# kdsuneraavinash/CH-Bin

Measured on AMD Instinct MI355X. Metric: convex-hull QP distances/sec (+ end-to-end bin-assign wall-clock), N=100000 D=136 B=64, higher is better.
Workload: dtype f64

## Files before the change

### ch-bin_amd/csrc/qp_kernels.hip

```cpp
#include "chb_internal.h"
#include "hull_solve16.h"
#include <cstdlib>
#include <type_traits>
#include <vector>

#include <math.h>

#include <algorithm>

#ifndef CHB_QP_UNROLL
#define CHB_QP_UNROLL 1
#endif

namespace chb {
namespace {


template <int M>
struct Sym {
    static constexpr int NP = M * (M + 1) / 2;
    __device__ static constexpr int at(int i, int j) { return i >= j ? i * (i + 1) / 2 + j : j * (j + 1) / 2 + i; }
};

template <int M>
__device__ __forceinline__ bool solve_affine(const double (&Q)[Sym<M>::NP], double s, unsigned S,
                                             double (&beta)[M])
{
    double L[M * (M - 1) / 2 + 1];
    double dg[M];
    bool ok = true;
#pragma unroll
    for (int k = 0; k < M; ++k) {
        const bool ink = (S >> k) & 1u;
        const double akk = ink ? Q[Sym<M>::at(k, k)] + s : 1.0;
        double dk = akk;
#pragma unroll
        for (int j = 0; j < k; ++j) dk -= L[k * (k - 1) / 2 + j] * L[k * (k - 1) / 2 + j] * dg[j];
        if (ink && !(dk > 1e-13 * akk)) ok = false;
        dg[k] = dk;
        const double inv = 1.0 / dk;
#pragma unroll
        for (int i = k + 1; i < M; ++i) {
            const bool ini = (S >> i) & 1u;
            double v = (ink && ini) ? Q[Sym<M>::at(i, k)] + s : 0.0;
#pragma unroll
            for (int j = 0; j < k; ++j) v -= L[i * (i - 1) / 2 + j] * L[k * (k - 1) / 2 + j] * dg[j];
            L[i * (i - 1) / 2 + k] = v * inv;
        }
    }
    if (!ok) return false;
    double z[M];
#pragma unroll
    for (int i = 0; i < M; ++i) {
        double v = ((S >> i) & 1u) ? 1.0 : 0.0;
#pragma unroll
        for (int j = 0; j < i; ++j) v -= L[i * (i - 1) / 2 + j] * z[j];
        z[i] = v;
    }
#pragma unroll
    for (int i = 0; i < M; ++i) z[i] = z[i] / dg[i];
    double sum = 0.0;
#pragma unroll
    for (int i = M - 1; i >= 0; --i) {
        double v = z[i];
#pragma unroll
        for (int j = i + 1; j < M; ++j) v -= L[j * (j - 1) / 2 + i] * beta[j];
        beta[i] = v;
        sum += v;
    }
    const double inv = 1.0 / sum;
#pragma unroll
    for (int i = 0; i < M; ++i) beta[i] *= inv;
    return sum > 0.0;
}

template <int M>
__device__ __forceinline__ double min_norm_point(const double (&Q)[Sym<M>::NP], int m,
                                                 double (&alpha)[M])
{
    double scale = 0.0;
    int i0 = 0;
    double best = kInf;
#pragma unroll
    for (int i = 0; i < M; ++i) {
        alpha[i] = 0.0;
        if (i < m) {
            const double qii = Q[Sym<M>::at(i, i)];
            scale = fmax(scale, qii);
            if (qii < best) { best = qii; i0 = i; }
        }
    }
    if (!(scale > 0.0)) {
#pragma unroll
        for (int i = 0; i < M; ++i) alpha[i] = (i == 0) ? 1.0 : 0.0;
        return scale == 0.0 ? 0.0 : scale;
    }
    unsigned S = 1u << i0, banned = 0u;
#pragma unroll
    for (int i = 0; i < M; ++i) alpha[i] = (i == i0) ? 1.0 : 0.0;
    const double tol = 1.4210854715202004e-14 * scale;

    for (int it = 0; it < 3 * M + 8; ++it) {
        double g[M];
        double val = 0.0;
#pragma unroll
        for (int i = 0; i < M; ++i) {
            double gi = 0.0;
#pragma unroll
            for (int j = 0; j < M; ++j) gi += Q[Sym<M>::at(i, j)] * alpha[j];
            g[i] = gi;
            val += alpha[i] * gi;
        }
        int jb = -1;
        double gmin = kInf;
#pragma unroll
        for (int i = 0; i < M; ++i)
            if (i < m && !(((S | banned) >> i) & 1u) && g[i] < gmin) { gmin = g[i]; jb = i; }
        if (jb < 0 || !(gmin < val - tol)) break;
        S |= 1u << jb;
        for (int mi = 0; mi <= M; ++mi) {
            double beta[M];
            if (!solve_affine<M>(Q, scale, S, beta)) {
                S &= ~(1u << jb);
                banned |= 1u << jb;
                break;
            }
            bool allpos = true;
#pragma unroll
            for (int i = 0; i < M; ++i)
                if (((S >> i) & 1u) && !(beta[i] > 0.0)) allpos = false;
            if (allpos) {
#pragma unroll
                for (int i = 0; i < M; ++i) alpha[i] = ((S >> i) & 1u) ? beta[i] : 0.0;
                break;
            }
            double theta = 1.0;
            int kr = -1;
#pragma unroll
            for (int i = 0; i < M; ++i)
                if (((S >> i) & 1u) && !(beta[i] > 0.0)) {
                    const double den = alpha[i] - beta[i];
                    const double r = den > 0.0 ? alpha[i] / den : 0.0;
                    if (kr < 0 || r < theta) { theta = r; kr = i; }
                }
#pragma unroll
            for (int i = 0; i < M; ++i) {
                const double v = alpha[i] + theta * (beta[i] - alpha[i]);
                alpha[i] = (((S >> i) & 1u) && i != kr) ? v : 0.0;
            }
            S &= ~(1u << kr);
            if (kr == jb) banned |= 1u << jb;
        }
    }
    double val = 0.0;
#pragma unroll
    for (int i = 0; i < M; ++i) {
        double gi = 0.0;
#pragma unroll
        for (int j = 0; j < M; ++j) gi += Q[Sym<M>::at(i, j)] * alpha[j];
        val += alpha[i] * gi;
    }
    return val;
}

template <int M>
__device__ __forceinline__ double affine_min_norm(const double (&Q)[Sym<M>::NP], int m, double (&alpha)[M])
{
    double scale = 0.0;
#pragma unroll
    for (int i = 0; i < M; ++i) {
        alpha[i] = 0.0;
        if (i < m) scale = fmax(scale, Q[Sym<M>::at(i, i)]);
    }
    if (!(scale > 0.0)) {
#pragma unroll
        for (int i = 0; i < M; ++i) alpha[i] = (i == 0) ? 1.0 : 0.0;
        return scale == 0.0 ? 0.0 : scale;
    }
    unsigned S = 0u;
    double beta[M];
#pragma unroll
    for (int k = 0; k < M; ++k) {
        if (k < m) {
            double trial[M];
            if (solve_affine<M>(Q, scale, S | (1u << k), trial)) {
                S |= 1u << k;
#pragma unroll
                for (int i = 0; i < M; ++i) beta[i] = trial[i];
            }
        }
    }
    if (S == 0u) {
#pragma unroll
        for (int i = 0; i < M; ++i) alpha[i] = (i == 0) ? 1.0 : 0.0;
        return Q[0];
    }
    double val = 0.0;
#pragma unroll
    for (int i = 0; i < M; ++i) alpha[i] = ((S >> i) & 1u) ? beta[i] : 0.0;
#pragma unroll
    for (int i = 0; i < M; ++i) {
        double gi = 0.0;
#pragma unroll
        for (int j = 0; j < M; ++j) gi += Q[Sym<M>::at(i, j)] * alpha[j];
        val += alpha[i] * gi;
    }
    return val;
}


__device__ __forceinline__ double reduce_scatter16(const double (&v)[16], int l16)
{
    double t8[8], t4[4], t2[2];
    const bool b8 = l16 & 8, b4 = l16 & 4, b2 = l16 & 2, b1 = l16 & 1;
#pragma unroll
    for (int e = 0; e < 8; ++e) t8[e] = (b8 ? v[e + 8] : v[e]) + __shfl_xor(b8 ? v[e] : v[e + 8], 8, 64);
#pragma unroll
    for (int e = 0; e < 4; ++e) t4[e] = (b4 ? t8[e + 4] : t8[e]) + __shfl_xor(b4 ? t8[e] : t8[e + 4], 4, 64);
#pragma unroll
    for (int e = 0; e < 2; ++e) t2[e] = (b2 ? t4[e + 2] : t4[e]) + __shfl_xor(b2 ? t4[e] : t4[e + 2], 2, 64);
    return (b1 ? t2[1] : t2[0]) + __shfl_xor(b1 ? t2[0] : t2[1], 1, 64);
}

template <int M, int WAVES, bool INDEXED>
__global__ __launch_bounds__(64 * WAVES, (M <= 5 ? 4 : 1)) void hull_qp_kernel(QpArgs a, int nprob, const int *xq,
                                                              const int *xhull, const int *xn,
                                                              int xm, double *xdist, double *xalpha, Gate gate)
{
    CHB_GATE(gate);
    constexpr int NP = Sym<M>::NP;
    static_assert(M <= 8, "m > 8 runs on hull_qp16_kernel");
    __shared__ double sQ[WAVES][NP][65];
    __shared__ int sN[WAVES][64];

    const int lane = threadIdx.x & 63, w = threadIdx.x >> 6;
    const int m = INDEXED ? xm : a.m;
    const int *act = INDEXED ? nullptr : a.active;
    if (act != nullptr) nprob = *a.n_active;
    const int npass = act != nullptr ? 1 : 16;
    const int ppw = 4 * npass;

    for (int g0 = (blockIdx.x * WAVES + w) * ppw; g0 < nprob; g0 += (int)gridDim.x * WAVES * ppw) {
    {
        const int grp = lane >> 4, l16 = lane & 15;
        for (int pass = 0; pass < npass; ++pass) {
            const int pl = pass * 4 + grp;
            const int g = g0 + pl;
            const bool valid = g < nprob;
            int n = 0, idm = -1, qid = 0;
            size_t slot = 0;
            if (valid) {
                if (INDEXED) {
                    qid = xq[g];
                    n = xn[g];
                    if (l16 < n) idm = xhull[(size_t)g * m + l16];
                } else {
                    const int pr = act ? act[g] : g;
                    const int pos = a.pos_begin + pr / a.B, c = pr - (pr / a.B) * a.B;
                    qid = a.bq[pos];
                    slot = (size_t)c * a.Kcap + pos;
                    n = a.lists.cnt[slot];
                    if (l16 < n) idm = a.lists.idx[slot * m + l16];
                }
            }
            bool changed = valid;
            if (!INDEXED && a.prev.idx != nullptr && act == nullptr && valid)
                changed = a.prev.cnt[slot] != n || (l16 < n && a.prev.idx[slot * m + l16] != idm);
            const bool doit = ((__ballot(changed) >> (16 * grp)) & 0xFFFFull) != 0ull;
            const double *vrow[M];
#pragma unroll
            for (int v = 0; v < M; ++v) {
                const int idv = __shfl(idm, 16 * grp + v, 64);
                vrow[v] = a.X + (size_t)(idv >= 0 ? idv : qid) * a.Dp;
            }
            if (!valid) continue;
            if (!doit) {
                if (l16 == 0) sN[w][pl] = -1;
                continue;
            }
            const double *xrow = a.X + (size_t)qid * a.Dp;
            double acc[NP];
#pragma unroll
            for (int e = 0; e < NP; ++e) acc[e] = 0.0;
            if (n > 0) {
                const int Dmain = a.Dp & ~31;
#pragma unroll CHB_QP_UNROLL
                for (int k = 2 * l16; k < Dmain; k += 32) {
                    const double2 xk = *reinterpret_cast<const double2 *>(xrow + k);
                    double2 y[M];
#pragma unroll
                    for (int v = 0; v < M; ++v) {
                        const double2 pv = *reinterpret_cast<const double2 *>(vrow[v] + k);
                        y[v] = double2{pv.x - xk.x, pv.y - xk.y};
                    }
#pragma unroll
                    for (int i = 0; i < M; ++i)
#pragma unroll
                        for (int j = 0; j <= i; ++j) {
                            double acc_ij = acc[Sym<M>::at(i, j)];
                            acc_ij = fma(y[i].x, y[j].x, acc_ij);
                            acc[Sym<M>::at(i, j)] = fma(y[i].y, y[j].y, acc_ij);
                        }
                }
                for (int k = Dmain + l16; k < a.Dp; k += 16) {
                    const double xk = xrow[k];
                    double y[M];
#pragma unroll
                    for (int v = 0; v < M; ++v) y[v] = vrow[v][k] - xk;
#pragma unroll
                    for (int i = 0; i < M; ++i)
#pragma unroll
                        for (int j = 0; j <= i; ++j) acc[Sym<M>::at(i, j)] = fma(y[i], y[j], acc[Sym<M>::at(i, j)]);
                }
            }
#pragma unroll
            for (int e0 = 0; e0 < NP; e0 += 16) {
                double v16[16];
#pragma unroll
                for (int e = 0; e < 16; ++e) v16[e] = e0 + e < NP ? acc[e0 + e] : 0.0;
                const double r = reduce_scatter16(v16, l16);
                if (e0 + l16 < NP) sQ[w][e0 + l16][pl] = r;
            }
            if (l16 == 0) sN[w][pl] = n;
        }
    }
    __builtin_amdgcn_wave_barrier();
    __builtin_amdgcn_s_waitcnt(0xC07F);

    const int g = g0 + lane;
    if (lane >= ppw || g >= nprob) continue;
    double Q[NP];
#pragma unroll
    for (int e = 0; e < NP; ++e) Q[e] = sQ[w][e][lane];
    const int n = sN[w][lane];
    if (n == -1) continue;
    double alpha[M];
    double dist;
    if (n <= 0) {
        dist = kInf;
#pragma unroll
        for (int v = 0; v < M; ++v) alpha[v] = 0.0;
    } else {
        const double val = a.metric == 0 ? min_norm_point<M>(Q, n, alpha) : affine_min_norm<M>(Q, n, alpha);
        dist = sqrt(fmax(val, 0.0));
    }
    if (INDEXED) {
        xdist[g] = dist;
        if (xalpha) {
#pragma unroll
            for (int v = 0; v < M; ++v)
                if (v < m) xalpha[(size_t)g * m + v] = alpha[v];
        }
    } else {
        const int pr = act ? act[g] : g;
        const int pos = a.pos_begin + pr / a.B, c = pr - (pr / a.B) * a.B;
        a.dist[(size_t)pos * a.B + c] = dist;
    }
    }
}

constexpr double kTieRel = 1e-11;

template <int CC, int NR, bool OFF32>
__device__ __forceinline__ void gram_rows(const double *X, int Dp, int Dk, int qid, int idm, int gbase, int l16,
                                          double (&r)[NR])
{
    constexpr int NP = CC * (CC + 1) / 2;
    static_assert(NP <= 16 * NR, "result registers");
    const char *Xb = reinterpret_cast<const char *>(X);
    const double *xrow = X + (size_t)qid * Dp;
    const unsigned xoff = (unsigned)qid * (unsigned)Dp * 8u;
    const double *vrow[OFF32 ? 1 : CC];
    unsigned voff[OFF32 ? CC : 1];
#pragma unroll
    for (int v = 0; v < CC; ++v) {
        const int idv = __shfl(idm, gbase + v, 64);
        if (OFF32) voff[v] = (unsigned)(idv >= 0 ? idv : qid) * (unsigned)Dp * 8u;
        else vrow[v] = X + (size_t)(idv >= 0 ? idv : qid) * Dp;
    }
    auto xat = [&](int k) { return OFF32 ? reinterpret_cast<const double *>(Xb + (size_t)(xoff + 8u * (unsigned)k)) : xrow + k; };
    auto vat = [&](int v, int k) {
        return OFF32 ? reinterpret_cast<const double *>(Xb + (size_t)(voff[OFF32 ? v : 0] + 8u * (unsigned)k)) : vrow[OFF32 ? 0 : v] + k;
    };
    double acc[NP];
#pragma unroll
    for (int e = 0; e < NP; ++e) acc[e] = 0.0;
    const int Dmain = Dk & ~31;
#pragma unroll 1
    for (int k = 2 * l16; k < Dmain; k += 32) {
        const double2 xk = *reinterpret_cast<const double2 *>(xat(k));
        double2 y[CC];
#pragma unroll
        for (int v = 0; v < CC; ++v) {
            const double2 pv = *reinterpret_cast<const double2 *>(vat(v, k));
            y[v] = double2{pv.x - xk.x, pv.y - xk.y};
        }
#pragma unroll
        for (int i = 0; i < CC; ++i)
#pragma unroll
            for (int j = 0; j <= i; ++j) {
                double t = acc[i * (i + 1) / 2 + j];
                t = fma(y[i].x, y[j].x, t);
                acc[i * (i + 1) / 2 + j] = fma(y[i].y, y[j].y, t);
            }
    }
    for (int k = Dmain + l16; k < Dk; k += 16) {
        const double xk = *xat(k);
        double y[CC];
#pragma unroll
        for (int v = 0; v < CC; ++v) y[v] = *vat(v, k) - xk;
#pragma unroll
        for (int i = 0; i < CC; ++i)
#pragma unroll
            for (int j = 0; j <= i; ++j) acc[i * (i + 1) / 2 + j] = fma(y[i], y[j], acc[i * (i + 1) / 2 + j]);
    }
#pragma unroll
    for (int t = 0; t < NR; ++t) {
        double v16[16];
#pragma unroll
        for (int e = 0; e < 16; ++e) v16[e] = 16 * t + e < NP ? acc[16 * t + e] : 0.0;
        r[t] = 16 * t < NP ? reduce_scatter16(v16, l16) : 0.0;
    }
}

#ifndef CHB_FUSED_C
#define CHB_FUSED_C 7
#endif
#ifndef CHB_FUSED_OCC
#define CHB_FUSED_OCC 3
#endif
#ifndef CHB_FUSED_WIDE
#define CHB_FUSED_WIDE 16
#endif
constexpr int kFusedWide = CHB_FUSED_WIDE;

template <bool OFF32>
__device__ __forceinline__ double diag_rows8(const double *X, int Dp, int Dk, int qid, int idm, int gbase, int l16, int v0)
{
    const char *Xb = reinterpret_cast<const char *>(X);
    const double *xrow = X + (size_t)qid * Dp;
    const unsigned xoff = (unsigned)qid * (unsigned)Dp * 8u;
    const double *vrow[OFF32 ? 1 : 8];
    unsigned voff[OFF32 ? 8 : 1];
#pragma unroll
    for (int v = 0; v < 8; ++v) {
        const int idv = __shfl(idm, gbase + v0 + v, 64);
        if (OFF32) voff[v] = (unsigned)(idv >= 0 ? idv : qid) * (unsigned)Dp * 8u;
        else vrow[v] = X + (size_t)(idv >= 0 ? idv : qid) * Dp;
    }
    auto xat = [&](int k) { return OFF32 ? reinterpret_cast<const double *>(Xb + (size_t)(xoff + 8u * (unsigned)k)) : xrow + k; };
    auto vat = [&](int v, int k) {
        return OFF32 ? reinterpret_cast<const double *>(Xb + (size_t)(voff[OFF32 ? v : 0] + 8u * (unsigned)k)) : vrow[OFF32 ? 0 : v] + k;
    };
    double acc[16];
#pragma unroll
    for (int e = 0; e < 16; ++e) acc[e] = 0.0;
    const int Dmain = Dk & ~31;
#pragma unroll 1
    for (int k = 2 * l16; k < Dmain; k += 32) {
        const double2 xk = *reinterpret_cast<const double2 *>(xat(k));
#pragma unroll
        for (int v = 0; v < 8; ++v) {
            const double2 pv = *reinterpret_cast<const double2 *>(vat(v, k));
            const double dx = pv.x - xk.x, dy = pv.y - xk.y;
            acc[v] = fma(dy, dy, fma(dx, dx, acc[v]));
        }
    }
    for (int k = Dmain + l16; k < Dk; k += 16) {
        const double xk = *xat(k);
#pragma unroll
        for (int v = 0; v < 8; ++v) {
            const double d = *vat(v, k) - xk;
            acc[v] = fma(d, d, acc[v]);
        }
    }
    return reduce_scatter16(acc, l16);
}

constexpr int kTrimMax = 32;
constexpr int kTrimKeep = 8;
constexpr int kNbTrimmed = -1;
constexpr double kTrimSlack = 1e-6;
constexpr double kTrimGamma = 2.5e-5;

__device__ __forceinline__ int trim_tail_col(int l16) { return 128 + 2 * l16; }

__device__ __forceinline__ double shadow_dot16(const unsigned short *Gs, int Dz, int qid, int ids, int nmax, int gbase, int l16,
                                               const uint4 &qm, unsigned qt)
{
    using f16x2 = __attribute__((ext_vector_type(2))) _Float16;
    auto dot2 = [](unsigned x, unsigned y, float c) {
        return __builtin_amdgcn_fdot2(__builtin_bit_cast(f16x2, x), __builtin_bit_cast(f16x2, y), c, false);
    };
    const int tcol = min(trim_tail_col(l16), Dz - 2);
    double acc[16];
#pragma unroll
    for (int v = 0; v < 16; ++v) acc[v] = 0.0;
#pragma unroll
    for (int v0 = 0; v0 < 16; v0 += 4) {
        if (v0 < nmax) {
#pragma unroll
            for (int v = v0; v < v0 + 4; ++v) {
                const int idv = __shfl(ids, gbase + v, 64);
                const unsigned short *row = Gs + (size_t)(idv >= 0 ? idv : qid) * Dz;
                const uint4 u = *reinterpret_cast<const uint4 *>(row + 8 * l16);
                const unsigned ut = *reinterpret_cast<const unsigned *>(row + tcol);
                acc[v] = (double)dot2(ut, qt, dot2(u.w, qm.w, dot2(u.z, qm.z, dot2(u.y, qm.y, dot2(u.x, qm.x, 0.f)))));
            }
        }
    }
    return reduce_scatter16(acc, l16);
}

__device__ __forceinline__ bool fused_pair_of(const FusedArgs &a, int g0, int lane, int nprob, int &pos, int &c)
{
    if (!a.stripe) {
        const int g = g0 + lane;
        pos = a.pos_begin + g / a.B;
        c = g - (g / a.B) * a.B;
        return g < nprob;
    }
    const int x = (int)(blockIdx.x & 7);
    const int nbx = (a.B - x + 7) >> 3;
    const int t = g0 + lane;
    const int pq = t / nbx;
    pos = a.pos_begin + pq;
    c = x + 8 * (t - pq * nbx);
    return pq < a.pos_end - a.pos_begin;
}

template <int M, int C, int WAVES, bool OFF32>
__global__ __launch_bounds__(64 * WAVES, CHB_FUSED_OCC) void hull_select_qp_kernel(FusedArgs a, int nprob, Gate gate)
{
    CHB_GATE(gate);
    constexpr int NPM = Sym<M>::NP;
    constexpr int NPC = C * (C + 1) / 2;
    constexpr int NR = (NPC + 15) / 16;
    constexpr int NCLS = C - M + 1;
    static_assert(C <= 8 && M <= C && C - M <= 3, "candidate Gram in registers");
    __shared__ double sQ[WAVES][NPM][65];
    __shared__ double sT[WAVES][4][NR * 16];
    __shared__ double sTh[WAVES][4][2];
    __shared__ int sSel[WAVES][4][16];
    __shared__ int sN[WAVES][64];
    __shared__ int sOrd[WAVES][64];
    __shared__ int sSlowN, sSlowBase;
    __shared__ int sTrim[WAVES][64][kTrimKeep];
    __shared__ int sTrimN[WAVES][64];
    __shared__ int sTrimCtr[3];

    const int lane = threadIdx.x & 63, w = threadIdx.x >> 6;
    const int grp = lane >> 4, l16 = lane & 15, gbase = lane & 48;
    const int m = a.m;
    const int Dk = (a.D + 7) & ~7;
    if (threadIdx.x == 0) sSlowN = 0;
    if (threadIdx.x < 3) sTrimCtr[threadIdx.x] = 0;
    __syncthreads();
    const int g0 = ((a.stripe ? (int)(blockIdx.x >> 3) : (int)blockIdx.x) * WAVES + w) * 64;
    unsigned long long slowmask = 0ull;
    int pos = 0, c = 0;
    bool valid = false;

    if (g0 < nprob) {
        valid = fused_pair_of(a, g0, lane, nprob, pos, c);
        int nb = 0, nu = 0, qid = 0;
        size_t slot = 0;
        bool changed = valid;
        if (valid) {
            qid = a.bq[pos];
            slot = (size_t)c * a.Kcap + pos;
            nb = a.cand_cnt[slot];
            if (a.candu != nullptr) nu = a.candu_cnt[slot];
            if (a.candp != nullptr && a.candp_cnt[slot] == nu) {
                if (nu == 0) changed = false;
                else if (nu <= 8) {
                    bool same = true;
                    for (int i = 0; i < nu; ++i) {
                        const int u = a.candu[slot * kCandCapU + i];
                        bool f = false;
                        for (int j = 0; j < nu; ++j) f = f || a.candp[slot * kCandCapU + j] == u;
                        same = same && f;
                    }
                    changed = !same;
                }
            }
        }
        if (a.short_cnt != nullptr) {
            bool sh = false;
            if (valid) sh = nb < min(m, a.bin_size != nullptr ? a.bin_size[c] : a.bin_ptr[c + 1] - a.bin_ptr[c]);
            const unsigned long long shm = __ballot(sh);
            if (shm != 0ull && lane == 0) atomicAdd(a.short_cnt, __popcll(shm));
        }
        int n = nb + nu;
        if (a.trim != nullptr) {
            const bool tr = changed && n > C && n <= kTrimMax;
            const unsigned long long tmask = __ballot(tr);
            const int ntrim = __popcll(tmask);
            if (ntrim > 0) {
                sTrimN[w][lane] = 0;
                if (tr) sOrd[w][__popcll(tmask & ((1ull << lane) - 1ull))] = lane;
                __builtin_amdgcn_wave_barrier();
                __builtin_amdgcn_s_waitcnt(0xC07F);
                const TrimArgs ta = *a.trim;
                auto mask32 = [](int nv) { return (unsigned)((1ull << min(max(16 * nv, 0), 32)) - 1ull); };
                const int nv = a.D - 8 * l16;
                const uint4 msk{mask32(nv), mask32(nv - 2), mask32(nv - 4), mask32(nv - 6)};
                const unsigned mskt = mask32(a.D - trim_tail_col(l16));
                int c_pairs = 0, c_in = 0, c_kept = 0;
                for (int p0 = 0; p0 < ntrim; p0 += 4) {
                    const int op = p0 + grp;
                    const bool has = op < ntrim;
                    const int pl = has ? sOrd[w][op] : 0;
                    const int n_s = __shfl(n, pl, 64);
                    const int n_g = has ? n_s : 0;
                    const int nb_g = __shfl(nb, pl, 64);
                    const int qid_g = __shfl(qid, pl, 64);
                    const size_t slot_g = (size_t)__shfl(c, pl, 64) * a.Kcap + (size_t)__shfl(pos, pl, 64);
                    int id0 = -1, id1 = -1;
                    if (l16 < n_g)
                        id0 = l16 < nb_g ? a.cand[slot_g * kCandCap + l16] : a.candu[slot_g * kCandCapU + (l16 - nb_g)];
                    if (16 + l16 < n_g)
                        id1 = 16 + l16 < nb_g ? a.cand[slot_g * kCandCap + 16 + l16] : a.candu[slot_g * kCandCapU + (16 + l16 - nb_g)];
                    bool bad = false;
                    if ((unsigned)id0 >= (unsigned)a.n_samples && id0 != -1) { bad = true; id0 = -1; }
                    if ((unsigned)id1 >= (unsigned)a.n_samples && id1 != -1) { bad = true; id1 = -1; }
                    int nmax = n_g;
                    nmax = max(nmax, __shfl_xor(nmax, 16, 64));
                    nmax = max(nmax, __shfl_xor(nmax, 32, 64));
                    nmax = __builtin_amdgcn_readfirstlane(nmax);
                    const unsigned short *qrow = ta.Gs + (size_t)qid_g * ta.Dz;
                    uint4 qm = *reinterpret_cast<const uint4 *>(qrow + 8 * l16);
                    qm.x &= msk.x; qm.y &= msk.y; qm.z &= msk.z; qm.w &= msk.w;
                    const unsigned qt = *reinterpret_cast<const unsigned *>(qrow + min(trim_tail_col(l16), ta.Dz - 2)) & mskt;
                    const float2 gj = ta.gq[qid_g];
                    const bool in0 = id0 >= 0, in1 = id1 >= 0;
                    const float2 g0 = ta.gq[in0 ? id0 : qid_g], g1 = ta.gq[in1 ? id1 : qid_g];
                    const double dot0 = shadow_dot16(ta.Gs, ta.Dz, qid_g, id0, nmax, gbase, l16, qm, qt);
                    double dot1 = 0.0;
                    if (nmax > 16) dot1 = shadow_dot16(ta.Gs, ta.Dz, qid_g, id1, nmax - 16, gbase, l16, qm, qt);
                    const double Nj = (double)gj.x, sNj = sqrt(Nj), flush = 0x1p-13 * sqrt((double)a.D);
                    auto bounds = [&](double dot, float2 gp, double &lo, double &hi) {
                        const double Np = (double)gp.x, sNp = sqrt(Np), rho = (double)gj.y + (double)gp.y;
                        const double T = Nj + Np - 2.0 * dot;
                        const double E = 2.0 * kTrimGamma * sNj * sNp + 0x1p-23 * (Nj + Np) + flush * (sNj + sNp) + 0x1p-27 * (double)a.D;
                        lo = sqrt(fmax(T - E, 0.0)) - rho;
                        hi = sqrt(T + E) + rho;
                    };
                    double lo0, lo1, hi0, hi1;
                    bounds(dot0, g0, lo0, hi0);
                    bounds(dot1, g1, lo1, hi1);
                    if (!in0) hi0 = kInf;
                    if (!in1) hi1 = kInf;
                    bad = bad || (in0 && !(hi0 < kInf)) || (in1 && !(hi1 < kInf));
                    int rank0 = 0, rank1 = 0;
#pragma unroll
                    for (int u = 0; u < 16; ++u) {
                        const double hu = __shfl(hi0, gbase + u, 64);
                        rank0 += (hu < hi0 || (hu == hi0 && u < l16)) ? 1 : 0;
                        rank1 += hu <= hi1 ? 1 : 0;
                    }
                    if (nmax > 16) {
#pragma unroll
                        for (int u = 0; u < 16; ++u) {
                            const double hu = __shfl(hi1, gbase + u, 64);
                            rank0 += hu < hi0 ? 1 : 0;
                            rank1 += (hu < hi1 || (hu == hi1 && u < l16)) ? 1 : 0;
                        }
                    }
                    double tau = (in0 && rank0 == m - 1) ? hi0 : (in1 && rank1 == m - 1) ? hi1 : kInf;
#pragma unroll
                    for (int off = 1; off < 16; off <<= 1) tau = fmin(tau, __shfl_xor(tau, off, 64));
                    const double lim = tau * (1.0 + kTrimSlack);
                    const bool k0 = in0 && !(lo0 > lim), k1 = in1 && !(lo1 > lim);
                    const unsigned badm = (unsigned)(__ballot(bad) >> gbase) & 0xffffu;
                    const unsigned b0 = (unsigned)(__ballot(k0) >> gbase) & 0xffffu, b1 = (unsigned)(__ballot(k1) >> gbase) & 0xffffu;
                    const int nk = badm != 0u ? n_g : __popc(b0) + __popc(b1);
                    if (has && badm == 0u && nk <= kTrimKeep) {
                        if (k0) sTrim[w][pl][__popc(b0 & ((1u << l16) - 1u))] = id0;
                        if (k1) sTrim[w][pl][__popc(b0) + __popc(b1 & ((1u << l16) - 1u))] = id1;
                        if (l16 == 0) sTrimN[w][pl] = nk;
                    }
                    if (has && l16 == 0) { c_pairs += 1; c_in += n_g; c_kept += nk; }
                }
                c_pairs += __shfl_xor(c_pairs, 16, 64); c_pairs += __shfl_xor(c_pairs, 32, 64);
                c_in += __shfl_xor(c_in, 16, 64); c_in += __shfl_xor(c_in, 32, 64);
                c_kept += __shfl_xor(c_kept, 16, 64); c_kept += __shfl_xor(c_kept, 32, 64);
                if (lane == 0) { atomicAdd(&sTrimCtr[0], c_pairs); atomicAdd(&sTrimCtr[1], c_in); atomicAdd(&sTrimCtr[2], c_kept); }
                __builtin_amdgcn_wave_barrier();
                __builtin_amdgcn_s_waitcnt(0xC07F);
                const int nt = sTrimN[w][lane];
                if (nt > 0) { n = nt; nb = kNbTrimmed; }
            }
        }
        int cls = 0;
        if (changed && n > 0) {
            if (n <= C) cls = n <= M ? 1 : n - M + 1;
            else if (n <= kFusedWide) cls = NCLS + 1;
        }
        slowmask = __ballot(changed && n > kFusedWide);
        sN[w][lane] = (changed && n == 0) ? 0 : -1;
        int before = 0, nwork = 0, nnarrow = 0;
#pragma unroll
        for (int k = 1; k <= NCLS + 1; ++k) {
            const unsigned long long mk = __ballot(cls == k);
            if (cls == k) before = nwork + __popcll(mk & ((1ull << lane) - 1ull));
            nwork += __popcll(mk);
            if (k == NCLS) nnarrow = nwork;
        }
        if (cls > 0) sOrd[w][before] = lane;
        __builtin_amdgcn_wave_barrier();
        __builtin_amdgcn_s_waitcnt(0xC07F);

        for (int p0 = 0; p0 < nnarrow; p0 += 4) {
            const int op = p0 + grp;
            const bool has = op < nnarrow;
            const int pl = has ? sOrd[w][op] : 0;
            const int n_s = __shfl(n, pl, 64);
            const int n_g = has ? n_s : 0;
            const int nb_g = __shfl(nb, pl, 64);
            const int qid_g = __shfl(qid, pl, 64);
            const size_t slot_g = (size_t)__shfl(c, pl, 64) * a.Kcap + (size_t)__shfl(pos, pl, 64);
            int idm = -1;
            if (l16 < n_g)
                idm = nb_g == kNbTrimmed ? sTrim[w][pl][l16]
                      : l16 < nb_g ? a.cand[slot_g * kCandCap + l16] : a.candu[slot_g * kCandCapU + (l16 - nb_g)];
            if ((unsigned)idm >= (unsigned)a.n_samples && idm != -1) {
                if (a.short_cnt != nullptr) atomicAdd(a.short_cnt, 1);
                idm = -1;
            }
            const int cw = __builtin_amdgcn_readfirstlane(__shfl(n, sOrd[w][min(p0 + 3, nnarrow - 1)], 64));
            double r[NR];
            if (cw <= M) gram_rows<M, NR, OFF32>(a.X, a.Dp, Dk, qid_g, idm, gbase, l16, r);
            else if (C >= M + 1 && cw == M + 1) gram_rows<(C >= M + 1 ? M + 1 : M), NR, OFF32>(a.X, a.Dp, Dk, qid_g, idm, gbase, l16, r);
            else if (C >= M + 2 && cw == M + 2) gram_rows<(C >= M + 2 ? M + 2 : M), NR, OFF32>(a.X, a.Dp, Dk, qid_g, idm, gbase, l16, r);
            else gram_rows<C, NR, OFF32>(a.X, a.Dp, Dk, qid_g, idm, gbase, l16, r);
            bool tie = false;
            if (has && n_g <= m) {
#pragma unroll
                for (int t = 0; t < NR; ++t)
                    if (16 * t + l16 < NPM) sQ[w][16 * t + l16][pl] = r[t];
                if (l16 == 0) sN[w][pl] = n_g;
            } else if (has) {
#pragma unroll
                for (int t = 0; t < NR; ++t) sT[w][grp][16 * t + l16] = r[t];
                __builtin_amdgcn_wave_barrier();
                __builtin_amdgcn_s_waitcnt(0xC07F);
                if (l16 < C) sSel[w][grp][8 + l16] = idm;
                __builtin_amdgcn_wave_barrier();
                __builtin_amdgcn_s_waitcnt(0xC07F);
                const double sv = l16 < n_g ? sT[w][grp][l16 * (l16 + 3) / 2] : kInf;
                int rank = 0;
#pragma unroll
                for (int u = 0; u < C; ++u) {
                    const double su = sT[w][grp][u * (u + 3) / 2];
                    const int iu = sSel[w][grp][8 + u];
                    rank += (u < n_g && u != l16 && (su < sv || (su == sv && iu < idm))) ? 1 : 0;
                }
                if (l16 < n_g) {
                    if (rank < m) sSel[w][grp][rank] = l16;
                    if (rank == m - 1) sTh[w][grp][0] = sv;
                    if (rank == m) sTh[w][grp][1] = sv;
                }
                __builtin_amdgcn_wave_barrier();
                __builtin_amdgcn_s_waitcnt(0xC07F);
                const double t0 = sTh[w][grp][0], t1 = sTh[w][grp][1];
                tie = !(t1 - t0 > kTieRel * t1);
                if (!tie) {
#pragma unroll
                    for (int t = 0; 16 * t < NPM; ++t) {
                        const int e = 16 * t + l16;
                        int i = 0;
#pragma unroll
                        for (int q = 1; q < M; ++q) i += (q * (q + 1) / 2 <= e) ? 1 : 0;
                        const int j = e - i * (i + 1) / 2;
                        if (e < NPM) {
                            double val = 0.0;
                            if (i < m) {
                                const int vi = sSel[w][grp][i], vj = sSel[w][grp][j];
                                const int hi = vi > vj ? vi : vj, lo = vi > vj ? vj : vi;
                                val = sT[w][grp][hi * (hi + 1) / 2 + lo];
                            }
                            sQ[w][e][pl] = val;
                        }
                    }
                    if (l16 == 0) sN[w][pl] = m;
                }
            }
            if (l16 == 0 && tie) slowmask |= 1ull << pl;
        }

        for (int p0 = nnarrow; p0 < nwork; p0 += 4) {
            const int op = p0 + grp;
            const bool has = op < nwork;
            const int pl = has ? sOrd[w][op] : 0;
            const int n_s = __shfl(n, pl, 64);
            const int n_g = has ? n_s : 0;
            const int nb_g = __shfl(nb, pl, 64);
            const int qid_g = __shfl(qid, pl, 64);
            const size_t slot_g = (size_t)__shfl(c, pl, 64) * a.Kcap + (size_t)__shfl(pos, pl, 64);
            int idm = -1;
            if (l16 < n_g)
                idm = nb_g == kNbTrimmed ? sTrim[w][pl][l16]
                      : l16 < nb_g ? a.cand[slot_g * kCandCap + l16] : a.candu[slot_g * kCandCapU + (l16 - nb_g)];
            if ((unsigned)idm >= (unsigned)a.n_samples && idm != -1) {
                if (a.short_cnt != nullptr) atomicAdd(a.short_cnt, 1);
                idm = -1;
            }
            int nmax = n_g;
            nmax = max(nmax, __shfl_xor(nmax, 16, 64));
            nmax = max(nmax, __shfl_xor(nmax, 32, 64));
            nmax = __builtin_amdgcn_readfirstlane(nmax);
            double sv = diag_rows8<OFF32>(a.X, a.Dp, Dk, qid_g, idm, gbase, l16, 0);
            if (nmax > 8) {
                const double s_hi = diag_rows8<OFF32>(a.X, a.Dp, Dk, qid_g, idm, gbase, l16, 8);
                const double moved = __shfl(s_hi, gbase + (l16 & 7), 64);
                sv = l16 < 8 ? sv : moved;
            }
            if (l16 >= n_g) sv = kInf;
            int rank = 0;
#pragma unroll
            for (int u = 0; u < 16; ++u) {
                const double su = __shfl(sv, gbase + u, 64);
                const int iu = __shfl(idm, gbase + u, 64);
                rank += (u < n_g && u != l16 && (su < sv || (su == sv && iu < idm))) ? 1 : 0;
            }
            if (has && l16 < n_g) {
                if (rank < m) sSel[w][grp][rank] = idm;
                if (rank == m - 1) sTh[w][grp][0] = sv;
                if (rank == m) sTh[w][grp][1] = sv;
            }
            __builtin_amdgcn_wave_barrier();
            __builtin_amdgcn_s_waitcnt(0xC07F);
            bool tie = false;
            int idm2 = -1;
            if (has) {
                const double t0 = sTh[w][grp][0], t1 = sTh[w][grp][1];
                tie = !(t1 - t0 > kTieRel * t1);
                if (l16 < m) idm2 = sSel[w][grp][l16];
            }
            double r[NR];
            gram_rows<M, NR, OFF32>(a.X, a.Dp, Dk, qid_g, idm2, gbase, l16, r);
            if (has && !tie) {
#pragma unroll
                for (int t = 0; t < NR; ++t)
                    if (16 * t + l16 < NPM) sQ[w][16 * t + l16][pl] = r[t];
                if (l16 == 0) sN[w][pl] = m;
            }
            if (l16 == 0 && tie) slowmask |= 1ull << pl;
        }
    }
    unsigned long long sm = slowmask;
    sm |= __shfl_xor(sm, 16, 64);
    sm |= __shfl_xor(sm, 32, 64);
    sm = __shfl(sm, 0, 64);
    __builtin_amdgcn_wave_barrier();
    __builtin_amdgcn_s_waitcnt(0xC07F);

    {
        const int n = valid ? sN[w][lane] : -1;
        if (valid && n != -1 && !((sm >> lane) & 1ull)) {
            double Q[NPM];
#pragma unroll
            for (int e = 0; e < NPM; ++e) Q[e] = sQ[w][e][lane];
            double alpha[M];
            double dist;
            if (n <= 0) {
                dist = kInf;
            } else {
                const double val = a.metric == 0 ? min_norm_point<M>(Q, n, alpha) : affine_min_norm<M>(Q, n, alpha);
                dist = sqrt(fmax(val, 0.0));
            }
            a.dist[(size_t)pos * a.B + c] = dist;
        }
    }

    const int nsl = __popcll(sm);
    int wbase = 0;
    if (lane == 0 && nsl > 0) wbase = atomicAdd(&sSlowN, nsl);
    __syncthreads();
    if (threadIdx.x == 0) sSlowBase = sSlowN > 0 ? atomicAdd(a.n_slow, sSlowN) : 0;
    if (threadIdx.x < 3 && a.trim != nullptr && sTrimCtr[0] > 0)
        atomicAdd(a.trim->ctr + threadIdx.x, (unsigned long long)sTrimCtr[threadIdx.x]);
    __syncthreads();
    wbase = __shfl(wbase, 0, 64) + sSlowBase;
    if (nsl > 0 && ((sm >> lane) & 1ull)) {
        const int before = __popcll(sm & ((1ull << lane) - 1ull));
        a.slow[wbase + before] = (pos - a.pos_begin) * a.B + c;
    }
}


#ifdef CHB_DEV_CLK
__device__ unsigned long long g_qp16_clk[131072][8];
#endif
#ifdef CHB_DEV_CLK
#define QP16_CLK(t) const unsigned long long t = __builtin_readcyclecounter()
#define QP16_CLK_ADD(i, v) do { if (lane == 0) atomicAdd(&g_qp16_stats[i], (unsigned long long)(v)); } while (0)
#define QP16_CLK_ACC(var, v) do { var += (unsigned long long)(v); } while (0)
#else
#define QP16_CLK(t) do { } while (0)
#define QP16_CLK_ADD(i, v) do { } while (0)
#define QP16_CLK_ACC(var, v) do { } while (0)
#endif

constexpr int kExtraMax = 2;
constexpr int kExtraNP = kExtraMax * (kExtraMax + 1) / 2;
#ifndef CHB_SW0
#define CHB_SW0 160
#define CHB_SW1 48
#define CHB_SW2 32
#endif
template <int NE, int CH, bool FULL>
__device__ __forceinline__ void gram_sweep16_chunk(const double *vptr, const double *const (&eptr)[kExtraMax],
                                                   const double *xs, int k0, int kq, int Dp, f64x4 &acc,
                                                   double (&ae)[kExtraMax], double (&ee)[kExtraNP])
{
    constexpr int NG = CH / 16;
    double2 v[NG][2], e[NE > 0 ? NE : 1][NG][2];
#pragma unroll
    for (int g = 0; g < NG; ++g) {
        const bool in = FULL || k0 + 16 * g + 4 * kq < Dp;
        v[g][0] = in ? *reinterpret_cast<const double2 *>(vptr + k0 + 16 * g) : double2{0.0, 0.0};
        v[g][1] = in ? *reinterpret_cast<const double2 *>(vptr + k0 + 16 * g + 2) : double2{0.0, 0.0};
#pragma unroll
        for (int b = 0; b < NE; ++b) {
            e[b][g][0] = in ? *reinterpret_cast<const double2 *>(eptr[b] + k0 + 16 * g) : double2{0.0, 0.0};
            e[b][g][1] = in ? *reinterpret_cast<const double2 *>(eptr[b] + k0 + 16 * g + 2) : double2{0.0, 0.0};
        }
    }
#pragma unroll
    for (int g = 0; g < NG; ++g) {
        if (FULL || k0 + 16 * g < Dp) {
            const double2 x0 = *reinterpret_cast<const double2 *>(xs + k0 + 16 * g + 4 * kq);
            const double2 x1 = *reinterpret_cast<const double2 *>(xs + k0 + 16 * g + 4 * kq + 2);
            const double y[4] = {v[g][0].x - x0.x, v[g][0].y - x0.y, v[g][1].x - x1.x, v[g][1].y - x1.y};
#pragma unroll
            for (int t = 0; t < 4; ++t) acc = __builtin_amdgcn_mfma_f64_16x16x4f64(y[t], y[t], acc, 0, 0, 0);
            double z[NE > 0 ? NE : 1][4];
#pragma unroll
            for (int b = 0; b < NE; ++b) {
                z[b][0] = e[b][g][0].x - x0.x; z[b][1] = e[b][g][0].y - x0.y;
                z[b][2] = e[b][g][1].x - x1.x; z[b][3] = e[b][g][1].y - x1.y;
#pragma unroll
                for (int t = 0; t < 4; ++t) ae[b] = fma(y[t], z[b][t], ae[b]);
#pragma unroll
                for (int b2 = 0; b2 <= b; ++b2)
#pragma unroll
                    for (int t = 0; t < 4; ++t) ee[b * (b + 1) / 2 + b2] = fma(z[b][t], z[b2][t], ee[b * (b + 1) / 2 + b2]);
            }
        }
    }
}
template <int NE, int CH>
__device__ __forceinline__ void gram_sweep16(const double *X, int Dp, int Dk, int q, int idv, const int (&ide)[kExtraMax], int kq,
                                             const double *xs, f64x4 &acc, double (&ae)[kExtraMax],
                                             double (&ee)[kExtraNP], int c0 = 0, bool first = true, bool last = true)
{
    const double *vptr = X + (size_t)(idv >= 0 ? idv : q) * Dp + 4 * kq + c0;
    const double *eptr[kExtraMax];
#pragma unroll
    for (int b = 0; b < kExtraMax; ++b) eptr[b] = X + (size_t)(b < NE ? ide[b] : q) * Dp + 4 * kq + c0;
    if (first) {
#pragma unroll
        for (int b = 0; b < kExtraMax; ++b) ae[b] = 0.0;
#pragma unroll
        for (int e = 0; e < kExtraNP; ++e) ee[e] = 0.0;
    }
    int k0 = 0;
    for (; k0 + CH <= Dk; k0 += CH) gram_sweep16_chunk<NE, CH, true>(vptr, eptr, xs, k0, kq, Dk, acc, ae, ee);
    if (k0 < Dk) gram_sweep16_chunk<NE, CH, false>(vptr, eptr, xs, k0, kq, Dk, acc, ae, ee);
    if (NE > 0 && last) {
#pragma unroll
        for (int b = 0; b < NE; ++b) {
            ae[b] += __shfl_xor(ae[b], 16, 64);
            ae[b] += __shfl_xor(ae[b], 32, 64);
        }
#pragma unroll
        for (int e = 0; e < NE * (NE + 1) / 2; ++e) {
            ee[e] += __shfl_xor(ee[e], 16, 64);
            ee[e] += __shfl_xor(ee[e], 32, 64);
        }
    }
}

template <bool INDEXED>
__global__ __launch_bounds__(256, CHB_QP16_OCC) void hull_qp16_kernel(QpArgs a, int nprob, const int *xq, const int *xhull,
                                                        const int *xn, int xm, double *xdist, double *xalpha, Gate gate)
{
    CHB_GATE(gate);
    __shared__ __attribute__((aligned(16))) double sQ[4][4][16][kQ16Ld];
    __shared__ __attribute__((aligned(16))) double sV[4][4][16];
    const int lane = threadIdx.x & 63, w = threadIdx.x >> 6;
    const int grp = lane >> 4, l16 = lane & 15;
    const int m = INDEXED ? xm : a.m;
    const int *act = INDEXED ? nullptr : a.active;
    if (act != nullptr) nprob = *a.n_active;
    for (int gw = (blockIdx.x * 4 + w) * 4; gw < nprob; gw += (int)gridDim.x * 16) {
        const int g = gw + grp;
        const bool valid = g < nprob;
        int n = 0, idm = -1, qid = 0, pr = 0;
        size_t slot = 0;
        if (valid) {
            if (INDEXED) {
                qid = xq[g];
                n = xn[g];
                if (l16 < n) idm = xhull[(size_t)g * m + l16];
            } else {
                pr = act ? act[g] : g;
                const int pos = a.pos_begin + pr / a.B, c = pr - (pr / a.B) * a.B;
                qid = a.bq[pos];
                slot = (size_t)c * a.Kcap + pos;
                n = a.lists.cnt[slot];
                if (l16 < n) idm = a.lists.idx[slot * m + l16];
            }
        }
        bool changed = valid;
        if (!INDEXED && a.prev.idx != nullptr && act == nullptr && valid)
            changed = a.prev.cnt[slot] != n || (l16 < n && a.prev.idx[slot * m + l16] != idm);
        const bool doit = ((__ballot(changed) >> (16 * grp)) & 0xFFFFull) != 0ull;

        const int row = lane & 15, kq = lane >> 4;
#pragma unroll 1
        for (int p = 0; p < 4; ++p) {
            const int np = __shfl(n, 16 * p, 64);
            const bool go = __shfl(doit ? 1 : 0, 16 * p, 64) != 0 && np > 0;
            const int id = __shfl(idm, 16 * p + row, 64);
            const int q = __shfl(qid, 16 * p, 64);
            if (!go) continue;
            f64x4 acc = {0.0, 0.0, 0.0, 0.0}, d0 = acc, d1 = acc;
            gram_tile16<false>(a.X, a.Dp, (a.D + 7) & ~7, q, id, -1, kq, acc, d0, d1);
#pragma unroll
            for (int r = 0; r < 4; ++r) sQ[w][p][kq + 4 * r][row] = acc[r];
        }
        __builtin_amdgcn_wave_barrier();
        __builtin_amdgcn_s_waitcnt(0xC07F);
        if (!valid || !doit) continue;

        double alpha = 0.0;
        const double val = n <= 0 ? kInf : solve16(&sQ[w][grp][0][0], &sV[w][grp][0], n, a.metric, lane, alpha);
        const double dist = n <= 0 ? kInf : sqrt(fmax(val, 0.0));
        if (INDEXED) {
            if (l16 == 0) xdist[g] = dist;
            if (xalpha && l16 < m) xalpha[(size_t)g * m + l16] = alpha;
        } else if (l16 == 0) {
            const int pos = a.pos_begin + pr / a.B, c = pr - (pr / a.B) * a.B;
            a.dist[(size_t)pos * a.B + c] = dist;
        }
    }
}

template <int WAVES, bool WIDEROW>
__global__ __launch_bounds__(64 * WAVES, CHB_QP16_OCC) void hull_select_qp16_kernel(FusedArgs a, int nprob, Gate gate)
{
    CHB_GATE(gate);
    __shared__ __attribute__((aligned(16))) double sQ[WAVES][4][16][kQ16Ld];
    __shared__ __attribute__((aligned(16))) double sV[WAVES][4][16];
    __shared__ __attribute__((aligned(16))) double sAE[WAVES][4][kExtraMax][16];
    __shared__ __attribute__((aligned(16))) double sEE[WAVES][4][kExtraNP];
    __shared__ __attribute__((aligned(16))) double sGD[WAVES][4][20];
    __shared__ __attribute__((aligned(16))) int sGI[WAVES][4][20];
    __shared__ __attribute__((aligned(16))) int sGN[WAVES][4][20];
    __shared__ double sTh[WAVES][4][2];
    __shared__ int sSlowN, sSlowBase;
    const int lane = threadIdx.x & 63, w = threadIdx.x >> 6;
    const int grp = lane >> 4, l16 = lane & 15;
    const int m = a.m;
    const int Dk = (a.D + 7) & ~7;
    constexpr bool widerow = WIDEROW;
    double *sDw = &sGD[w][0][0];
    int *sIdw = &sGI[w][0][0], *sNeww = &sGN[w][0][0];
    if (threadIdx.x == 0) sSlowN = 0;
    __syncthreads();
    const int gw = ((a.stripe ? (int)(blockIdx.x >> 3) : (int)blockIdx.x) * WAVES + w) * 4;
    int pos = 0, c = 0;
    const bool valid = fused_pair_of(a, gw, grp, nprob, pos, c);
    int nb = 0, nu = 0, qid = 0;
    bool changed = valid;
    const size_t slot = (size_t)c * a.Kcap + pos;
    if (valid) {
        qid = a.bq[pos];
        nb = a.cand_cnt[slot];
        if (a.candu != nullptr) nu = a.candu_cnt[slot];
        if (a.candp != nullptr && a.candp_cnt[slot] == nu) {
            bool same = true;
            for (int i = l16; i < nu; i += 16) {
                const int u = a.candu[slot * kCandCapU + i];
                bool f = false;
                for (int j = 0; j < nu; ++j) f = f || a.candp[slot * kCandCapU + j] == u;
                same = same && f;
            }
            changed = ((__ballot(!same) >> (lane & 48)) & 0xFFFFull) != 0ull;
        }
    }
    if (a.short_cnt != nullptr && valid && l16 == 0 &&
        nb < min(m, a.bin_size != nullptr ? a.bin_size[c] : a.bin_ptr[c + 1] - a.bin_ptr[c]))
        atomicAdd(a.short_cnt, 1);
    QP16_CLK(tc0);
#ifdef CHB_DEV_CLK
    unsigned long long c_ids = 0, c_sweep = 0, c_one = 0;
#endif
    const int n = nb + nu;
    const bool work = changed && n > 0 && n <= 32;
    bool slow = changed && n > 32;
    int nsel = n < m ? n : m;

// ... 593 lines not shown
```

Measured before the change: 683.3 million.

## Warm-start simplex QP from full active set and stage narrow candidate ids in LDS

The small simplex QP solver now starts from the full support with uniform weights and first tries a direct affine solve over all vertices, falling back to the single-vertex start if that solve fails. This is meant to skip most active-set iterations when the optimum is interior. Separately, when a problem has few candidates, their ids are copied once into an LDS list, so the narrow Gram passes read ids from LDS instead of doing scattered global loads from the cand and candu arrays. The risks are extra solve work when the full-support guess is poor, and the added static_assert that C must not exceed the LDS list size.

```diff
diff --git a/ch-bin_amd/csrc/qp_kernels.hip b/ch-bin_amd/csrc/qp_kernels.hip
--- a/ch-bin_amd/csrc/qp_kernels.hip
+++ b/ch-bin_amd/csrc/qp_kernels.hip
@@ -95,32 +95,41 @@
         for (int i = 0; i < M; ++i) alpha[i] = (i == 0) ? 1.0 : 0.0;
         return scale == 0.0 ? 0.0 : scale;
     }
-    unsigned S = 1u << i0, banned = 0u;
-#pragma unroll
-    for (int i = 0; i < M; ++i) alpha[i] = (i == i0) ? 1.0 : 0.0;
+    unsigned S = (1u << m) - 1u, banned = 0u;
+    const double uni = 1.0 / (double)m;
+#pragma unroll
+    for (int i = 0; i < M; ++i) alpha[i] = i < m ? uni : 0.0;
     const double tol = 1.4210854715202004e-14 * scale;
 
-    for (int it = 0; it < 3 * M + 8; ++it) {
-        double g[M];
-        double val = 0.0;
-#pragma unroll
-        for (int i = 0; i < M; ++i) {
-            double gi = 0.0;
-#pragma unroll
-            for (int j = 0; j < M; ++j) gi += Q[Sym<M>::at(i, j)] * alpha[j];
-            g[i] = gi;
-            val += alpha[i] * gi;
-        }
+    for (int it = -1; it < 3 * M + 8; ++it) {
         int jb = -1;
-        double gmin = kInf;
-#pragma unroll
-        for (int i = 0; i < M; ++i)
-            if (i < m && !(((S | banned) >> i) & 1u) && g[i] < gmin) { gmin = g[i]; jb = i; }
-        if (jb < 0 || !(gmin < val - tol)) break;
-        S |= 1u << jb;
+        if (it >= 0) {
+            double g[M];
+            double val = 0.0;
+#pragma unroll
+            for (int i = 0; i < M; ++i) {
+                double gi = 0.0;
+#pragma unroll
+                for (int j = 0; j < M; ++j) gi += Q[Sym<M>::at(i, j)] * alpha[j];
+                g[i] = gi;
+                val += alpha[i] * gi;
+            }
+            double gmin = kInf;
+#pragma unroll
+            for (int i = 0; i < M; ++i)
+                if (i < m && !(((S | banned) >> i) & 1u) && g[i] < gmin) { gmin = g[i]; jb = i; }
+            if (jb < 0 || !(gmin < val - tol)) break;
+            S |= 1u << jb;
+        }
         for (int mi = 0; mi <= M; ++mi) {
             double beta[M];
             if (!solve_affine<M>(Q, scale, S, beta)) {
+                if (jb < 0) {
+                    S = 1u << i0;
+#pragma unroll
+                    for (int i = 0; i < M; ++i) alpha[i] = (i == i0) ? 1.0 : 0.0;
+                    break;
+                }
                 S &= ~(1u << jb);
                 banned |= 1u << jb;
                 break;
@@ -130,8 +139,9 @@
             for (int i = 0; i < M; ++i)
                 if (((S >> i) & 1u) && !(beta[i] > 0.0)) allpos = false;
             if (allpos) {
-#pragma unroll
-                for (int i = 0; i < M; ++i) alpha[i] = ((S >> i) & 1u) ? beta[i] : 0.0;
+                const bool one = jb < 0 && (S & (S - 1u)) == 0u;
+#pragma unroll
+                for (int i = 0; i < M; ++i) alpha[i] = ((S >> i) & 1u) ? (one ? 1.0 : beta[i]) : 0.0;
                 break;
             }
             double theta = 1.0;
@@ -479,7 +489,7 @@
 
 constexpr int kTrimMax = 32;
 constexpr int kTrimKeep = 8;
-constexpr int kNbTrimmed = -1;
+constexpr int kNbInLds = -1;
 constexpr double kTrimSlack = 1e-6;
 constexpr double kTrimGamma = 2.5e-5;
 
@@ -538,6 +548,7 @@
     constexpr int NR = (NPC + 15) / 16;
     constexpr int NCLS = C - M + 1;
     static_assert(C <= 8 && M <= C && C - M <= 3, "candidate Gram in registers");
+    static_assert(C <= kTrimKeep, "the narrow passes take their ids from the LDS list");
     __shared__ double sQ[WAVES][NPM][65];
     __shared__ double sT[WAVES][4][NR * 16];
     __shared__ double sTh[WAVES][4][2];
@@ -545,7 +556,7 @@
     __shared__ int sN[WAVES][64];
     __shared__ int sOrd[WAVES][64];
     __shared__ int sSlowN, sSlowBase;
-    __shared__ int sTrim[WAVES][64][kTrimKeep];
+    __shared__ int sIds[WAVES][64][kTrimKeep];
     __shared__ int sTrimN[WAVES][64];
     __shared__ int sTrimCtr[3];
 
@@ -676,8 +687,8 @@
                     const unsigned b0 = (unsigned)(__ballot(k0) >> gbase) & 0xffffu, b1 = (unsigned)(__ballot(k1) >> gbase) & 0xffffu;
                     const int nk = badm != 0u ? n_g : __popc(b0) + __popc(b1);
                     if (has && badm == 0u && nk <= kTrimKeep) {
-                        if (k0) sTrim[w][pl][__popc(b0 & ((1u << l16) - 1u))] = id0;
-                        if (k1) sTrim[w][pl][__popc(b0) + __popc(b1 & ((1u << l16) - 1u))] = id1;
+                        if (k0) sIds[w][pl][__popc(b0 & ((1u << l16) - 1u))] = id0;
+                        if (k1) sIds[w][pl][__popc(b0) + __popc(b1 & ((1u << l16) - 1u))] = id1;
                         if (l16 == 0) sTrimN[w][pl] = nk;
                     }
                     if (has && l16 == 0) { c_pairs += 1; c_in += n_g; c_kept += nk; }
@@ -689,8 +700,14 @@
                 __builtin_amdgcn_wave_barrier();
                 __builtin_amdgcn_s_waitcnt(0xC07F);
                 const int nt = sTrimN[w][lane];
-                if (nt > 0) { n = nt; nb = kNbTrimmed; }
-            }
+                if (nt > 0) { n = nt; nb = kNbInLds; }
+            }
+        }
+        if (changed && nb != kNbInLds && n > 0 && n <= kTrimKeep) {
+#pragma unroll
+            for (int i = 0; i < kTrimKeep; ++i)
+                if (i < n) sIds[w][lane][i] = i < nb ? a.cand[slot * kCandCap + i] : a.candu[slot * kCandCapU + (i - nb)];
+            nb = kNbInLds;
         }
         int cls = 0;
         if (changed && n > 0) {
@@ -717,13 +734,9 @@
             const int pl = has ? sOrd[w][op] : 0;
             const int n_s = __shfl(n, pl, 64);
             const int n_g = has ? n_s : 0;
-            const int nb_g = __shfl(nb, pl, 64);
             const int qid_g = __shfl(qid, pl, 64);
-            const size_t slot_g = (size_t)__shfl(c, pl, 64) * a.Kcap + (size_t)__shfl(pos, pl, 64);
             int idm = -1;
-            if (l16 < n_g)
-                idm = nb_g == kNbTrimmed ? sTrim[w][pl][l16]
-                      : l16 < nb_g ? a.cand[slot_g * kCandCap + l16] : a.candu[slot_g * kCandCapU + (l16 - nb_g)];
+            if (l16 < n_g) idm = sIds[w][pl][l16];
             if ((unsigned)idm >= (unsigned)a.n_samples && idm != -1) {
                 if (a.short_cnt != nullptr) atomicAdd(a.short_cnt, 1);
                 idm = -1;
@@ -800,7 +813,7 @@
             const size_t slot_g = (size_t)__shfl(c, pl, 64) * a.Kcap + (size_t)__shfl(pos, pl, 64);
             int idm = -1;
             if (l16 < n_g)
-                idm = nb_g == kNbTrimmed ? sTrim[w][pl][l16]
+                idm = nb_g == kNbInLds ? sIds[w][pl][l16]
                       : l16 < nb_g ? a.cand[slot_g * kCandCap + l16] : a.candu[slot_g * kCandCapU + (l16 - nb_g)];
             if ((unsigned)idm >= (unsigned)a.n_samples && idm != -1) {
                 if (a.short_cnt != nullptr) atomicAdd(a.short_cnt, 1);
```

Measured after the change: 703.6 million, median of 6. 1.03x the previous value.
